# zhaotudou/HeteroFusionRCNN

Hardware: AMD Instinct MI355X
Metric: KITTI frames/sec RPN train step (higher is better)
Workload: dtype f32

## Files before the change

heterofusionrcnn_amd/csrc/xconv_common.h:

```cpp
#pragma once
#include "hf_common.h"

#include <initializer_list>

namespace hf {

template <int M>
__device__ __forceinline__ void store_m(float *base, size_t elem, const float (&v)[M])
{
    float *p = base + elem;
    if constexpr (M == 4 || M == 8) {
        if ((reinterpret_cast<uintptr_t>(base) & 15) == 0) {
#pragma unroll
            for (int q = 0; q < M / 4; ++q) reinterpret_cast<float4 *>(p)[q] = make_float4(v[4 * q], v[4 * q + 1], v[4 * q + 2], v[4 * q + 3]);
            return;
        }
    } else if constexpr (M == 2) {
        if ((reinterpret_cast<uintptr_t>(base) & 7) == 0) { *reinterpret_cast<float2 *>(p) = make_float2(v[0], v[1]); return; }
    }
#pragma unroll
    for (int m = 0; m < M; ++m) p[m] = v[m];
}
template <int M>
__device__ __forceinline__ void load_m(const float *base, size_t elem, float (&v)[M])
{
    const float *p = base + elem;
    if constexpr (M == 4 || M == 8) {
        if ((reinterpret_cast<uintptr_t>(base) & 15) == 0) {
#pragma unroll
            for (int q = 0; q < M / 4; ++q) {
                const float4 t = reinterpret_cast<const float4 *>(p)[q];
                v[4 * q] = t.x; v[4 * q + 1] = t.y; v[4 * q + 2] = t.z; v[4 * q + 3] = t.w;
            }
            return;
        }
    } else if constexpr (M == 2) {
        if ((reinterpret_cast<uintptr_t>(base) & 7) == 0) { const float2 t = *reinterpret_cast<const float2 *>(p); v[0] = t.x; v[1] = t.y; return; }
    }
#pragma unroll
    for (int m = 0; m < M; ++m) v[m] = p[m];
}


constexpr int kXcThreads = 256;

typedef float f2 __attribute__((ext_vector_type(2)));

struct XcPair {
    const float *base;
    unsigned hi;
    bool gathered, live, hi_live;
};

__device__ __forceinline__ XcPair xc_pair(int ch, int c, int c0, const float *f, const float *fts, bool gather)
{
    XcPair s;
    s.live = ch < c;
    s.hi_live = ch + 1 < c;
    const int cc = s.live ? ch : (c - 1) & ~1;
    s.hi = s.hi_live ? 1u : 0u;
    s.gathered = gather && cc >= c0;
    s.base = s.gathered ? fts + (cc - c0) : f + cc;
    return s;
}

template <bool V2>
__device__ __forceinline__ f2 ld_pair(const float *p, unsigned hi)
{
    if constexpr (V2) return *reinterpret_cast<const f2 *>(p);
    else return f2{p[0], p[hi]};
}

template <int M, bool V2>
__device__ __forceinline__ void st_pair_m(float *p, bool hi_live, const f2 (&v)[M])
{
    if constexpr (V2) {
#pragma unroll
        for (int q = 0; q < M; ++q) {
            const int e0 = 2 * q, e1 = 2 * q + 1;
            reinterpret_cast<f2 *>(p)[q] = f2{e0 < M ? v[e0].x : v[e0 - M].y, e1 < M ? v[e1].x : v[e1 - M].y};
        }
    } else {
#pragma unroll
        for (int m = 0; m < M; ++m) p[m] = v[m].x;
        if (hi_live) {
#pragma unroll
            for (int m = 0; m < M; ++m) p[M + m] = v[m].y;
        }
    }
}

constexpr int kXcRows = 2;

struct XcCloud {
    long long next;
    unsigned tbase;
};

__device__ __forceinline__ unsigned xc_tbase(XcCloud &cl, long long r, int rows_per_cloud, int n_src)
{
    while (r >= cl.next) { cl.next += rows_per_cloud; cl.tbase += static_cast<unsigned>(n_src); }
    return cl.tbase;
}

__device__ __forceinline__ XcCloud xc_cloud(long long r, int rows_per_cloud, int n_src)
{
    const long long b = r / rows_per_cloud;
    return XcCloud{(b + 1) * rows_per_cloud, static_cast<unsigned>(b * n_src)};
}

template <int K, bool GATHER, bool V2>
__device__ __forceinline__ void xc_gather_row(const XcPair &s, long long r, unsigned tbase, const int *__restrict__ idx,
                                              unsigned lstride, unsigned c1, f2 (&fv)[K])
{
    const unsigned rk = static_cast<unsigned>(r) * K;
#pragma unroll
    for (int j = 0; j < K; ++j) {
        const unsigned lo = (rk + j) * lstride;
        unsigned off = lo;
        if constexpr (GATHER) {
            const unsigned go = (tbase + static_cast<unsigned>(idx[rk + j])) * c1;
            off = s.gathered ? go : lo;
        }
        fv[j] = ld_pair<V2>(s.base + off, s.hi);
    }
}

template <int K>
struct XcXRows {
    static constexpr int KK = K * K, Q = (KK + 63) / 64;
    float v[kXcRows][Q];
    __device__ __forceinline__ void load(const float *__restrict__ x, const long long (&rr)[kXcRows], int lane)
    {
#pragma unroll
        for (int i = 0; i < kXcRows; ++i)
#pragma unroll
            for (int q = 0; q < Q; ++q) {
                const int p = lane + 64 * q;
                v[i][q] = x[rr[i] * KK + (p < KK ? p : KK - 1)];
            }
    }
    __device__ __forceinline__ void stage(float (*xs)[KK], int lane) const
    {
        __builtin_amdgcn_fence(__ATOMIC_SEQ_CST, "wavefront");
        __builtin_amdgcn_wave_barrier();
#pragma unroll
        for (int i = 0; i < kXcRows; ++i)
#pragma unroll
            for (int q = 0; q < Q; ++q)
                if (lane + 64 * q < KK) xs[i][lane + 64 * q] = v[i][q];
        __builtin_amdgcn_fence(__ATOMIC_SEQ_CST, "wavefront");
        __builtin_amdgcn_wave_barrier();
    }
};

struct XcSource {
    const float *base;
    long long stride;
    bool gathered;
};

__device__ __forceinline__ XcSource xc_source(int ch, int c, int c0, const float *f, const float *fts, const int *idx)
{
    XcSource s;
    if (idx == nullptr) { s.base = f + ch; s.stride = c; s.gathered = false; }
    else if (ch - (ch & 63) < c0) { s.base = f + ch; s.stride = c0; s.gathered = false; }
    else { s.base = fts + (ch - c0); s.stride = c - c0; s.gathered = true; }
    return s;
}


template <int K, int M, bool GATHER, bool V2, bool BN>
__global__ __launch_bounds__(kXcThreads) void xconv_dw_fwd_kernel(long long rows, int c, int c0, int rows_per_block,
                                                                 const float *__restrict__ x, const float *__restrict__ f,
                                                                 const float *__restrict__ gamma, const float *__restrict__ beta,
                                                                 const float *__restrict__ mean, const float *__restrict__ invstd,
                                                                 const float *__restrict__ fts, const int *__restrict__ idx, int n_src,
                                                                 int rows_per_cloud, const float *__restrict__ wd, float *__restrict__ out)
{
    static_assert(GATHER || !BN, "the BatchNorm fold exists on the gather route only");
    const int lane = threadIdx.x & 63, wave = __builtin_amdgcn_readfirstlane(static_cast<int>(threadIdx.x >> 6));
    const int ch = blockIdx.y * 128 + 2 * lane;
    const XcPair src = xc_pair(ch, c, c0, f, fts, GATHER);
    const int cw = src.live ? ch : (c - 1) & ~1;
    f2 w[K][M];
#pragma unroll
    for (int k = 0; k < K; ++k)
#pragma unroll
        for (int m = 0; m < M; ++m) w[k][m] = f2{wd[(static_cast<size_t>(k) * c + cw) * M + m], wd[(static_cast<size_t>(k) * c + cw + src.hi) * M + m]};
    bool some_lifted = false;
    f2 ba, bmu, bb;
    if constexpr (BN) {
        const int cb = src.gathered ? 0 : cw;
        some_lifted = static_cast<int>(blockIdx.y) * 128 < c0;
        ba = f2{gamma[cb] * invstd[cb], gamma[cb + 1] * invstd[cb + 1]};
        bmu = f2{mean[cb], mean[cb + 1]};
        bb = f2{beta[cb], beta[cb + 1]};
    }
    const unsigned lstride = GATHER ? c0 : c, c1 = c - c0;
    const long long r0 = static_cast<long long>(blockIdx.x) * rows_per_block;
    const long long r1 = r0 + rows_per_block < rows ? r0 + rows_per_block : rows;
    __shared__ float xs[kXcThreads / 64][kXcRows][K * K];
    XcCloud cl = xc_cloud(r0, rows_per_cloud, n_src);
    for (long long rb = r0 + wave; rb < r1; rb += 4 * kXcRows) {
        f2 fv[kXcRows][K];
        long long rr[kXcRows];
#pragma unroll
        for (int i = 0; i < kXcRows; ++i) rr[i] = rb + 4 * i < r1 ? rb + 4 * i : r1 - 1;
        XcXRows<K> xrow;
        xrow.load(x, rr, lane);
#pragma unroll
        for (int i = 0; i < kXcRows; ++i) {
            const unsigned tb = GATHER ? xc_tbase(cl, rr[i], rows_per_cloud, n_src) : 0u;
            xc_gather_row<K, GATHER, V2>(src, rr[i], tb, idx, lstride, c1, fv[i]);
        }
        xrow.stage(xs[wave], lane);
#pragma unroll
        for (int i = 0; i < kXcRows; ++i) {
            if (rb + 4 * i >= r1) break;
            if constexpr (BN) {
                if (some_lifted) {
#pragma unroll
                    for (int j = 0; j < K; ++j) {
                        const f2 z = fv[i][j];
                        const f2 h = ba * (f2{elu_stream(z.x), elu_stream(z.y)} - bmu) + bb;
                        fv[i][j] = src.gathered ? z : h;
                    }
                }
            }
            const float *xr = xs[wave][i];
            f2 o[M];
#pragma unroll
            for (int m = 0; m < M; ++m) o[m] = f2{0.f, 0.f};
#pragma unroll
            for (int k = 0; k < K; ++k) {
                f2 t = xr[k * K] * fv[i][0];
#pragma unroll
                for (int j = 1; j < K; ++j) t = t + xr[k * K + j] * fv[i][j];
#pragma unroll
                for (int m = 0; m < M; ++m) o[m] = o[m] + t * w[k][m];
            }
            if (src.live) st_pair_m<M, V2>(out + static_cast<size_t>(rr[i] * c + ch) * M, src.hi_live, o);
        }
    }
}

template <int K, int M, bool GATHER, bool BN>
__global__ __launch_bounds__(kXcThreads) __attribute__((amdgpu_waves_per_eu(BN ? 4 : 1))) void xconv_dw_bwd_fw_kernel(
    long long rows, int c, int c0, int rows_per_block, const float *__restrict__ x, const float *__restrict__ f,
    const float *__restrict__ gamma, const float *__restrict__ beta, const float *__restrict__ mean, const float *__restrict__ invstd,
    const float *__restrict__ fts, const int *__restrict__ idx, int n_src, int rows_per_cloud, const float *__restrict__ wd,
    const float *__restrict__ grad_out, float *__restrict__ grad_f, float *__restrict__ grad_gathered, float *__restrict__ grad_wd,
    float *__restrict__ wd_partial, float *__restrict__ bn_partial)
{
    static_assert(GATHER || !BN, "the BatchNorm fold exists on the gather route only");
    const int lane = threadIdx.x & 63, wave = __builtin_amdgcn_readfirstlane(static_cast<int>(threadIdx.x >> 6));
    const int ch = blockIdx.y * 64 + lane;
    const bool live = ch < c;
    const XcSource src = xc_source(live ? ch : blockIdx.y * 64, c, c0, f, fts, GATHER ? idx : nullptr);
    if (GATHER && src.gathered && !grad_wd && !grad_gathered) return;
    bool lifted = false;
    float bis, ba, bmu, bb, s1 = 0.f, s2 = 0.f;
    if constexpr (BN) {
        lifted = static_cast<int>(blockIdx.y) * 64 < c0;
        const int cb = lifted ? ch : 0;
        bis = invstd[cb]; ba = gamma[cb] * bis; bmu = mean[cb]; bb = beta[cb];
    }
    float w[K][M], gw[K][M];
#pragma unroll
    for (int k = 0; k < K; ++k)
#pragma unroll
        for (int m = 0; m < M; ++m) { w[k][m] = live ? wd[(static_cast<size_t>(k) * c + ch) * M + m] : 0.f; gw[k][m] = 0.f; }
    const long long r0 = static_cast<long long>(blockIdx.x) * rows_per_block;
    const long long r1 = r0 + rows_per_block < rows ? r0 + rows_per_block : rows;
    for (long long r = r0 + wave; r < r1; r += kXcThreads / 64) {
        const float *xr = x + r * (K * K);
        float fv[K], xv[K], g[M], gfx[K];
        const long long tbase = (GATHER && src.gathered) ? static_cast<long long>(static_cast<unsigned>(r) / static_cast<unsigned>(rows_per_cloud)) * n_src : 0;
#pragma unroll
        for (int j = 0; j < K; ++j) {
            const long long srow = (GATHER && src.gathered) ? tbase + idx[r * K + j] : r * K + j;
            fv[j] = live ? src.base[srow * src.stride] : 0.f;
            if constexpr (BN) xv[j] = 0.f;
        }
        if constexpr (BN) {
            if (lifted) {
#pragma unroll
                for (int j = 0; j < K; ++j) {
                    xv[j] = elu_stream(fv[j]);
                    fv[j] = ba * (xv[j] - bmu) + bb;
                }
            }
        }
        load_m<M>(grad_out, static_cast<size_t>(r * c + (live ? ch : 0)) * M, g);
        if (!live) {
#pragma unroll
            for (int m = 0; m < M; ++m) g[m] = 0.f;
        }
#pragma unroll
        for (int k = 0; k < K; ++k) {
            float a = 0.f;
#pragma unroll
            for (int m = 0; m < M; ++m) a = a + g[m] * w[k][m];
            gfx[k] = a;
            float t = xr[k * K] * fv[0];
#pragma unroll
            for (int j = 1; j < K; ++j) t = t + xr[k * K + j] * fv[j];
#pragma unroll
            for (int m = 0; m < M; ++m) gw[k][m] = gw[k][m] + t * g[m];
        }
        float *gdst = (GATHER && src.gathered) ? (grad_gathered ? grad_gathered + (ch - c0) : nullptr) : (grad_f ? grad_f + ch : nullptr);
        if (live && gdst) {
            float ga[K];
#pragma unroll
            for (int j = 0; j < K; ++j) {
                float a = xr[j] * gfx[0];
#pragma unroll
                for (int k = 1; k < K; ++k) a = a + xr[k * K + j] * gfx[k];
                gdst[(r * K + j) * src.stride] = a;
                ga[j] = a;
            }
            if constexpr (BN) {
                if (lifted) {
#pragma unroll
                    for (int j = 0; j < K; ++j) { s1 += ga[j]; s2 += ga[j] * ((xv[j] - bmu) * bis); }
                }
            }
        }
    }
    __shared__ float red[K * M][64];
    if constexpr (BN) {
        if (lifted && grad_f) {
            for (int wv = 0; wv < kXcThreads / 64; ++wv) {
                if (wave == wv) {
                    red[0][lane] = wv == 0 ? s1 : red[0][lane] + s1;
                    red[1][lane] = wv == 0 ? s2 : red[1][lane] + s2;
                }
                __syncthreads();
            }
            if (wave == 0) {
                float *mine = bn_partial + static_cast<size_t>(blockIdx.x) * 2 * c0;
                mine[ch] = red[0][lane];
                mine[c0 + ch] = red[1][lane];
            }
        }
    }
    if (grad_wd) {
        for (int wv = 0; wv < kXcThreads / 64; ++wv) {
            if (wave == wv && live) {
#pragma unroll
                for (int k = 0; k < K; ++k)
#pragma unroll
                    for (int m = 0; m < M; ++m) red[k * M + m][lane] = wv == 0 ? gw[k][m] : red[k * M + m][lane] + gw[k][m];
            }
            __syncthreads();
        }
        float *mine = (BN || wd_partial) ? wd_partial + static_cast<size_t>(blockIdx.x) * K * c * M : nullptr;
        for (int i = threadIdx.x; i < K * M * 64; i += kXcThreads) {
            const int km = i >> 6, c2 = blockIdx.y * 64 + (i & 63);
            if (c2 < c) {
                const size_t e = (static_cast<size_t>(km / M) * c + c2) * M + km % M;
                if (BN || mine) mine[e] = red[km][i & 63];
                else atomicAdd(&grad_wd[e], red[km][i & 63]);
            }
        }
    }
}


template <int M>
__device__ __forceinline__ void xc_load_m(const float *arg, const float *p, float (&v)[M])
{
    if constexpr (M == 4) {
        if ((reinterpret_cast<uintptr_t>(arg) & 15) == 0) {
            const float4 t = *reinterpret_cast<const float4 *>(p);
            v[0] = t.x; v[1] = t.y; v[2] = t.z; v[3] = t.w;
            return;
        }
    } else if constexpr (M == 2) {
        if ((reinterpret_cast<uintptr_t>(arg) & 7) == 0) { const float2 t = *reinterpret_cast<const float2 *>(p); v[0] = t.x; v[1] = t.y; return; }
    }
#pragma unroll
    for (int m = 0; m < M; ++m) v[m] = p[m];
}

struct XcCloudDiv {
    long long first, next;
    long long tbase;
};

__device__ __forceinline__ long long xc_tbase_div(XcCloudDiv &cl, long long r, int rows_per_cloud, int n_src)
{
    if (r >= cl.next || r < cl.first) {
        const long long b = static_cast<long long>(static_cast<unsigned>(r) / static_cast<unsigned>(rows_per_cloud));
        cl.first = b * rows_per_cloud;
        cl.next = cl.first + rows_per_cloud;
        cl.tbase = b * n_src;
    }
    return cl.tbase;
}

template <int CTRL>
__device__ __forceinline__ float xc_dpp(float v)
{
    return __int_as_float(__builtin_amdgcn_update_dpp(0, __float_as_int(v), CTRL, 0xf, 0xf, true));
}

template <int KK, int OFF, int N>
__device__ __forceinline__ void xc_lane_fold(float (&v)[KK], int lane)
{
    static_assert(N == 64 || N == 16, "chunks of 64 or 16 entries");
    typedef unsigned u2 __attribute__((ext_vector_type(2)));
#pragma unroll
    for (int i = 0; i < N / 2; ++i) {
        const u2 s = __builtin_amdgcn_permlane32_swap(__float_as_uint(v[OFF + i]), __float_as_uint(v[OFF + i + N / 2]), false, false);
        v[OFF + i] = __uint_as_float(s.x) + __uint_as_float(s.y);
    }
#pragma unroll
    for (int i = 0; i < N / 4; ++i) {
        const u2 s = __builtin_amdgcn_permlane16_swap(__float_as_uint(v[OFF + i]), __float_as_uint(v[OFF + i + N / 4]), false, false);
        v[OFF + i] = __uint_as_float(s.x) + __uint_as_float(s.y);
    }
    const bool b3 = (lane & 8) != 0, b2 = (lane & 4) != 0;
#pragma unroll
    for (int i = 0; i < N / 8; ++i) {
        const float lo = v[OFF + i], hi = v[OFF + i + N / 8];
        v[OFF + i] = (b3 ? hi : lo) + xc_dpp<0x128>(b3 ? lo : hi);
    }
#pragma unroll
    for (int i = 0; i < N / 16; ++i) {
        const float lo = v[OFF + i], hi = v[OFF + i + N / 16];
        v[OFF + i] = (b2 ? hi : lo) + xc_dpp<0x141>(b2 ? lo : hi);
    }
    if constexpr (N == 64) {
        const bool b1 = (lane & 2) != 0, b0 = (lane & 1) != 0;
#pragma unroll
        for (int i = 0; i < 2; ++i) {
            const float lo = v[OFF + i], hi = v[OFF + i + 2];
            v[OFF + i] = (b1 ? hi : lo) + xc_dpp<0x4e>(b1 ? lo : hi);
        }
        const float lo = v[OFF], hi = v[OFF + 1];
        v[OFF] = (b0 ? hi : lo) + xc_dpp<0xb1>(b0 ? lo : hi);
    } else {
        v[OFF] = v[OFF] + xc_dpp<0x4e>(v[OFF]);
        v[OFF] = v[OFF] + xc_dpp<0xb1>(v[OFF]);
    }
}

template <int KK, int OFF = 0>
__device__ __forceinline__ void xc_store_dx(float (&acc)[KK], int lane, float *__restrict__ dst)
{
    static_assert((KK - OFF) % 64 == 0 || (KK - OFF) % 64 == 16, "K * K is a multiple of 64, or 16 more");
    if constexpr (KK - OFF >= 64) {
        xc_lane_fold<KK, OFF, 64>(acc, lane);
        dst[OFF + lane] = acc[OFF];
        xc_store_dx<KK, OFF + 64>(acc, lane, dst);
    } else if constexpr (KK - OFF == 16) {
        xc_lane_fold<KK, OFF, 16>(acc, lane);
        if ((lane & 3) == 0) dst[OFF + (lane >> 2)] = acc[OFF];
    }
}

__device__ __forceinline__ const float *xc_at(const float *base, unsigned byte_off)
{
    return reinterpret_cast<const float *>(reinterpret_cast<const char *>(base) + byte_off);
}

constexpr int kXcWdSlots = 64;
inline __host__ __device__ bool xc_bwd_x_fast(int c, int km) { return ((c + 63) >> 6) * km <= kXcWdSlots; }
inline size_t xc_bwd_x_lds_bytes(int c, int c0_bn, int km)
{
    return xc_bwd_x_fast(c, km) ? sizeof(float) * (64 * static_cast<size_t>((c + 63) >> 6) * km + 3 * static_cast<size_t>(c0_bn)) : 0;
}

template <int K, int M>
struct XcTrip {
    float fv[K], g[M];
};

template <int K, int M, bool GATHER, bool BN, bool FAST>
__device__ __forceinline__ void xc_bwd_x_rows(long long rows, int c, int c0, const float *__restrict__ f,
                                              const float *__restrict__ gamma, const float *__restrict__ beta,
                                              const float *__restrict__ mean, const float *__restrict__ invstd,
                                              const float *__restrict__ fts, const int *__restrict__ idx, int n_src, int rows_per_cloud,
                                              const float *__restrict__ wd, const float *__restrict__ grad_out,
                                              float *__restrict__ grad_x, float *lds)
{
    constexpr int KK = K * K, KM = K * M;
    const int lane = threadIdx.x & 63, w = __builtin_amdgcn_readfirstlane(static_cast<int>(threadIdx.x >> 6));
    const long long wave = w + static_cast<long long>(blockIdx.x) * (kXcThreads / 64);
    const long long nwaves = static_cast<long long>(gridDim.x) * (kXcThreads / 64);
    const int trips = (c + 63) >> 6, c1 = c - c0;
    const unsigned lstride = GATHER ? c0 : c;
    float *bnl = lds + trips * KM * 64;
    if constexpr (FAST) {
        for (int i = threadIdx.x; i < trips * KM * 64; i += kXcThreads) {
            const int l = i & 63, s = i >> 6, t = s / KM, km = s - t * KM, ch = 64 * t + l;
            lds[i] = ch < c ? wd[(static_cast<size_t>(km / M) * c + ch) * M + km % M] : 0.f;
        }
        if constexpr (BN) {
            for (int i = threadIdx.x; i < c0; i += kXcThreads) {
                bnl[i] = gamma[i] * invstd[i];
                bnl[c0 + i] = mean[i];
                bnl[2 * c0 + i] = beta[i];
            }
        }
        __syncthreads();
    }
    if (wave >= rows) return;

    int nidx[K];
    auto load_idx = [&](long long r) {
        if constexpr (GATHER) {
            const long long rc = r < rows ? r : rows - 1;
#pragma unroll
            for (int j = 0; j < K; ++j) nidx[j] = idx[rc * K + j];
        }
    };
    XcCloudDiv cl{0, 0, 0};
    const float *fl = f, *go = grad_out, *tj[K];
    auto set_row = [&](long long r) {
        fl = f + r * K * static_cast<long long>(lstride);
        go = grad_out + r * c * static_cast<long long>(M);
        if constexpr (GATHER) {
            const long long tb = xc_tbase_div(cl, r, rows_per_cloud, n_src);
#pragma unroll
            for (int j = 0; j < K; ++j) tj[j] = fts + static_cast<unsigned long long>(tb + nidx[j]) * static_cast<unsigned>(c1);
        }
    };
    auto load_trip = [&](int t, XcTrip<K, M> &o) {
        const int ch = 64 * t + lane;
        const unsigned cc = ch < c ? ch : c - 1;
        const float *bj[K];
        unsigned sub = 0;
        if (GATHER && 64 * t >= c0) {
            sub = c0;
#pragma unroll
            for (int j = 0; j < K; ++j) bj[j] = tj[j];
        } else {
#pragma unroll
            for (int j = 0; j < K; ++j) bj[j] = fl + j * static_cast<size_t>(lstride);
        }
        const unsigned off = (cc - sub) * 4u;
#pragma unroll
        for (int j = 0; j < K; ++j) o.fv[j] = *xc_at(bj[j], off);
        xc_load_m<M>(grad_out, xc_at(go, cc * (4u * M)), o.g);
    };

    long long r = wave;
    int t = 0;
    load_idx(r);
    set_row(r);
    XcTrip<K, M> cur, nxt;
    load_trip(0, cur);
    static_assert(K % 2 == 0, "pairs of j");
    f2 acc[K][K / 2];
    for (;;) {
        const bool last = t + 1 == trips;
        const long long rn = last ? r + nwaves : r;
        const int tn = last ? 0 : t + 1;
        const bool more = rn < rows;
        if (t == 0) load_idx(r + nwaves);
        if (last) set_row(more ? rn : r);
        load_trip(tn, nxt);
        const int ch = 64 * t + lane;
        const bool live = ch < c;
        const unsigned cc = live ? ch : c - 1;
        if (BN && 64 * t < c0) {
            float ba, bmu, bb;
            if constexpr (FAST) { ba = bnl[cc]; bmu = bnl[c0 + cc]; bb = bnl[2 * c0 + cc]; }
            else { ba = gamma[cc] * invstd[cc]; bmu = mean[cc]; bb = beta[cc]; }
#pragma unroll
            for (int j = 0; j < K; ++j) cur.fv[j] = ba * (elu_stream(cur.fv[j]) - bmu) + bb;
        }
        f2 ap[K / 2];
        {
            const float *wt = lds + (t * KM * 64 + lane);
            auto wv = [&](int k, int m) { return FAST ? wt[(k * M + m) * 64] : wd[(static_cast<size_t>(k) * c + cc) * M + m]; };
#pragma unroll
            for (int i = 0; i < K / 2; ++i) {
                ap[i] = cur.g[0] * f2{wv(2 * i, 0), wv(2 * i + 1, 0)};
#pragma unroll
                for (int m = 1; m < M; ++m) ap[i] = ap[i] + cur.g[m] * f2{wv(2 * i, m), wv(2 * i + 1, m)};
            }
        }
        f2 fp[K / 2];
#pragma unroll
        for (int i = 0; i < K / 2; ++i) fp[i] = f2{cur.fv[2 * i], cur.fv[2 * i + 1]};
        if (t == 0) {
            if (live) {
#pragma unroll
                for (int k = 0; k < K; ++k)
#pragma unroll
                    for (int i = 0; i < K / 2; ++i) acc[k][i] = ap[k / 2][k % 2] * fp[i];
            } else {
#pragma unroll
                for (int k = 0; k < K; ++k)
#pragma unroll
                    for (int i = 0; i < K / 2; ++i) acc[k][i] = f2{0.f, 0.f};
            }
        } else if (live) {
#pragma unroll
            for (int k = 0; k < K; ++k) {
                f2 p[K / 2];
#pragma unroll
                for (int i = 0; i < K / 2; ++i) p[i] = ap[k / 2][k % 2] * fp[i];
                __builtin_amdgcn_sched_barrier(0);
#pragma unroll
                for (int i = 0; i < K / 2; ++i) acc[k][i] = acc[k][i] + p[i];
                __builtin_amdgcn_sched_barrier(0);
            }
        }
        if (last) {
            float flat[KK];
#pragma unroll
            for (int k = 0; k < K; ++k)
#pragma unroll
                for (int i = 0; i < K / 2; ++i) { flat[k * K + 2 * i] = acc[k][i].x; flat[k * K + 2 * i + 1] = acc[k][i].y; }
            xc_store_dx<KK>(flat, lane, grad_x + r * KK);
        }
        if (!more) break;
        cur = nxt;
        r = rn;
        t = tn;
    }
}

template <int K, int M, bool GATHER, bool BN>
__device__ __forceinline__ void xc_bwd_x_body(long long rows, int c, int c0, const float *__restrict__ f,
                                              const float *__restrict__ gamma, const float *__restrict__ beta,
                                              const float *__restrict__ mean, const float *__restrict__ invstd,
                                              const float *__restrict__ fts, const int *__restrict__ idx, int n_src, int rows_per_cloud,
                                              const float *__restrict__ wd, const float *__restrict__ grad_out,
                                              float *__restrict__ grad_x, float *lds)
{
    if (xc_bwd_x_fast(c, K * M))
        xc_bwd_x_rows<K, M, GATHER, BN, true>(rows, c, c0, f, gamma, beta, mean, invstd, fts, idx, n_src, rows_per_cloud, wd, grad_out, grad_x, lds);
    else
        xc_bwd_x_rows<K, M, GATHER, BN, false>(rows, c, c0, f, gamma, beta, mean, invstd, fts, idx, n_src, rows_per_cloud, wd, grad_out, grad_x, lds);
}

void xdw_pair_grid(long long rows, int c, dim3 &grid, int &rpb, int blocks_per_cu);
void xdw_bwd_grid(long long rows, int c, dim3 &grid, int &rpb);
bool xdw_offsets_fit(long long rows, int k, int c, long long src_rows);
bool xdw_v2(int c, std::initializer_list<const void *> ptrs);
bool xdw_fts_direct(long long rows, int n_src, int rows_per_cloud, int k, int c1, int m);
size_t xdw_gathered_bytes(int b, int rows_per_cloud, int k, int c1);
int xdw_table_grad(long long src_rows, int n_src, int rows_per_cloud, int k, int c, int c0, int m, const float *x, const float *wd,
                   const float *grad_out, const int *offsets, const int *entries, float *grad_fts, hipStream_t st);

struct XdwGradPlan {
    bool direct;
    float *gathered;
    float *wd_partial;
};
XdwGradPlan xdw_grad_plan(int b, int n_src, int rows_per_cloud, int k, int c1, int m, const float *grad_fts, void *workspace);
int xdw_grad_table(const XdwGradPlan &plan, int b, int n_src, int rows_per_cloud, int k, int c0, int c1, int m, const float *x,
                   const float *wd, const float *grad_out, const int *offsets, const int *entries, float *grad_fts, hf_stream_t stream);
int xdw_grad_empty(int b, int n_src, int k, int c0, int c1, int m, float *grad_fts, float *grad_wd, hipStream_t st);

}
```

Baseline: 332.3.

## Restructure depthwise weight-grad backward kernel with LDS-staged X and prefetched row batches

Rewrites the xconv depthwise backward (weight/feature grad) kernel so each wave stages its X matrices into LDS in paired layout. It processes k in pairs with packed f2 math, software-pipelines the gathered feature, index and grad_out loads one batch ahead, and uses scalar base pointers with unsigned lane offsets. Large K*M configurations keep weights in LDS, and the occupancy hint is raised to 4 waves/EU for all variants. The aim is to hide gather latency and cut address arithmetic and VGPR pressure, at the cost of extra LDS traffic, more complex code and possible register spills.

```diff
diff --git a/heterofusionrcnn_amd/csrc/xconv_common.h b/heterofusionrcnn_amd/csrc/xconv_common.h
--- a/heterofusionrcnn_amd/csrc/xconv_common.h
+++ b/heterofusionrcnn_amd/csrc/xconv_common.h
@@ -2,6 +2,7 @@
 #include "hf_common.h"
 
 #include <initializer_list>
+#include <type_traits>
 
 namespace hf {
 
@@ -103,6 +104,16 @@
     return cl.tbase;
 }
 
+__device__ __forceinline__ unsigned xc_tbase_step(XcCloud &cl, long long r, int rows_per_cloud, int n_src)
+{
+    while (r >= cl.next) {
+        cl.next += rows_per_cloud;
+        cl.tbase += static_cast<unsigned>(n_src);
+        asm volatile("" : "+s"(cl.tbase));
+    }
+    return cl.tbase;
+}
+
 __device__ __forceinline__ XcCloud xc_cloud(long long r, int rows_per_cloud, int n_src)
 {
     const long long b = r / rows_per_cloud;
@@ -168,6 +179,73 @@
     else { s.base = fts + (ch - c0); s.stride = c - c0; s.gathered = true; }
     return s;
 }
+
+__device__ __forceinline__ const float *xc_at(const float *base, unsigned byte_off)
+{
+    return reinterpret_cast<const float *>(reinterpret_cast<const char *>(base) + byte_off);
+}
+
+typedef __attribute__((address_space(1))) float xc_gfloat;
+__device__ __forceinline__ xc_gfloat *xc_sbase(const float *p)
+{
+    const unsigned long long b = reinterpret_cast<unsigned long long>(p);
+    unsigned lo = __builtin_amdgcn_readfirstlane(static_cast<unsigned>(b)), hi = __builtin_amdgcn_readfirstlane(static_cast<unsigned>(b >> 32));
+    asm("" : "+s"(lo), "+s"(hi));
+    return (xc_gfloat *)((static_cast<unsigned long long>(hi) << 32) | lo);
+}
+__device__ __forceinline__ unsigned xc_lane_off(unsigned off)
+{
+    asm volatile("" : "+v"(off));
+    return off;
+}
+__device__ __forceinline__ xc_gfloat *xc_gat(xc_gfloat *base, unsigned byte_off)
+{
+    return (xc_gfloat *)((__attribute__((address_space(1))) char *)base + byte_off);
+}
+
+template <int M>
+__device__ __forceinline__ void xc_load_m(const float *arg, const float *p, float (&v)[M])
+{
+    if constexpr (M == 4) {
+        if ((reinterpret_cast<uintptr_t>(arg) & 15) == 0) {
+            const float4 t = *reinterpret_cast<const float4 *>(p);
+            v[0] = t.x; v[1] = t.y; v[2] = t.z; v[3] = t.w;
+            return;
+        }
+    } else if constexpr (M == 2) {
+        if ((reinterpret_cast<uintptr_t>(arg) & 7) == 0) { const float2 t = *reinterpret_cast<const float2 *>(p); v[0] = t.x; v[1] = t.y; return; }
+    }
+#pragma unroll
+    for (int m = 0; m < M; ++m) v[m] = p[m];
+}
+
+template <int M>
+__device__ __forceinline__ void xc_gload_m(const float *arg, xc_gfloat *p, float (&v)[M])
+{
+    typedef float v4 __attribute__((ext_vector_type(4)));
+    if constexpr (M == 4) {
+        if ((reinterpret_cast<uintptr_t>(arg) & 15) == 0) {
+            const v4 t = *(__attribute__((address_space(1))) v4 *)p;
+            v[0] = t.x; v[1] = t.y; v[2] = t.z; v[3] = t.w;
+            return;
+        }
+    } else if constexpr (M == 2) {
+        if ((reinterpret_cast<uintptr_t>(arg) & 7) == 0) { const f2 t = *(__attribute__((address_space(1))) f2 *)p; v[0] = t.x; v[1] = t.y; return; }
+    }
+#pragma unroll
+    for (int m = 0; m < M; ++m) v[m] = p[m];
+}
+
+template <int K, int M, int R>
+struct XcFwBatch {
+    static constexpr int Q = (K * K + 63) / 64;
+    float x[R][Q];
+    f2 fv[R][K / 2];
+    float g[R][M];
+};
+constexpr int xc_fw_rows(int k, int m, bool bn) { return k * m >= 24 ? 1 : kXcRows; }
+constexpr bool xc_fw_wd_lds(int k, int m) { return k * m >= 32; }
+constexpr bool xc_fw_pipe(int k, int m, bool bn) { return k == 4 || k * m <= 8; }
 
 
 template <int K, int M, bool GATHER, bool V2, bool BN>
@@ -246,7 +324,7 @@
 }
 
 template <int K, int M, bool GATHER, bool BN>
-__global__ __launch_bounds__(kXcThreads) __attribute__((amdgpu_waves_per_eu(BN ? 4 : 1))) void xconv_dw_bwd_fw_kernel(
+__global__ __launch_bounds__(kXcThreads) __attribute__((amdgpu_waves_per_eu(4))) void xconv_dw_bwd_fw_kernel(
     long long rows, int c, int c0, int rows_per_block, const float *__restrict__ x, const float *__restrict__ f,
     const float *__restrict__ gamma, const float *__restrict__ beta, const float *__restrict__ mean, const float *__restrict__ invstd,
     const float *__restrict__ fts, const int *__restrict__ idx, int n_src, int rows_per_cloud, const float *__restrict__ wd,
@@ -254,6 +332,7 @@
     float *__restrict__ wd_partial, float *__restrict__ bn_partial)
 {
     static_assert(GATHER || !BN, "the BatchNorm fold exists on the gather route only");
+    constexpr int R = xc_fw_rows(K, M, BN), Q = XcFwBatch<K, M, R>::Q;
     const int lane = threadIdx.x & 63, wave = __builtin_amdgcn_readfirstlane(static_cast<int>(threadIdx.x >> 6));
     const int ch = blockIdx.y * 64 + lane;
     const bool live = ch < c;
@@ -266,69 +345,178 @@
         const int cb = lifted ? ch : 0;
         bis = invstd[cb]; ba = gamma[cb] * bis; bmu = mean[cb]; bb = beta[cb];
     }
-    float w[K][M], gw[K][M];
-#pragma unroll
-    for (int k = 0; k < K; ++k)
-#pragma unroll
-        for (int m = 0; m < M; ++m) { w[k][m] = live ? wd[(static_cast<size_t>(k) * c + ch) * M + m] : 0.f; gw[k][m] = 0.f; }
+    static_assert(K % 2 == 0, "pairs of k");
+    constexpr bool WL = xc_fw_wd_lds(K, M);
+    __shared__ float red[K * M][64];
+    f2 *const wl = reinterpret_cast<f2 *>(&red[0][0]) + lane * M;
+    f2 w[WL ? 1 : K / 2][M], gw[K / 2][M];
+#pragma unroll
+    for (int kp = 0; kp < K / 2; ++kp)
+#pragma unroll
+        for (int m = 0; m < M; ++m) {
+            const f2 wk = live ? f2{wd[(static_cast<size_t>(2 * kp) * c + ch) * M + m], wd[(static_cast<size_t>(2 * kp + 1) * c + ch) * M + m]} : f2{0.f, 0.f};
+            if constexpr (WL) { if (wave == 0) wl[kp * 64 * M + m] = wk; }
+            else w[kp][m] = wk;
+            gw[kp][m] = f2{0.f, 0.f};
+        }
+    if constexpr (WL) __syncthreads();
     const long long r0 = static_cast<long long>(blockIdx.x) * rows_per_block;
     const long long r1 = r0 + rows_per_block < rows ? r0 + rows_per_block : rows;
-    for (long long r = r0 + wave; r < r1; r += kXcThreads / 64) {
-        const float *xr = x + r * (K * K);
-        float fv[K], xv[K], g[M], gfx[K];
-        const long long tbase = (GATHER && src.gathered) ? static_cast<long long>(static_cast<unsigned>(r) / static_cast<unsigned>(rows_per_cloud)) * n_src : 0;
-#pragma unroll
-        for (int j = 0; j < K; ++j) {
-            const long long srow = (GATHER && src.gathered) ? tbase + idx[r * K + j] : r * K + j;
-            fv[j] = live ? src.base[srow * src.stride] : 0.f;
-            if constexpr (BN) xv[j] = 0.f;
-        }
+    const bool gathered = GATHER && static_cast<int>(blockIdx.y) * 64 >= c0;
+    const int cc = live ? ch : c - 1;
+    const unsigned stride = static_cast<unsigned>(GATHER ? (gathered ? c - c0 : c0) : c);
+    const unsigned foff = static_cast<unsigned>(gathered ? cc - c0 : cc) * 4u, goff = static_cast<unsigned>(cc) * (4u * M);
+    unsigned xoff[Q];
+#pragma unroll
+    for (int q = 0; q < Q; ++q) xoff[q] = static_cast<unsigned>(lane + 64 * q < K * K ? lane + 64 * q : K * K - 1) * 4u;
+    float *const gdst = gathered ? grad_gathered : grad_f;
+    __shared__ float xs[kXcThreads / 64][R][2][K * K];
+    unsigned xpos[Q];
+#pragma unroll
+    for (int q = 0; q < Q; ++q) {
+        const int e = lane + 64 * q < K * K ? lane + 64 * q : K * K - 1, k = e / K, j = e - k * K;
+        xpos[q] = ((k >> 1) * K + j) * 2 + (k & 1);
+    }
+    auto stage = [&](const float (&xr)[R][Q]) {
+        __builtin_amdgcn_fence(__ATOMIC_SEQ_CST, "wavefront");
+        __builtin_amdgcn_wave_barrier();
+#pragma unroll
+        for (int i = 0; i < R; ++i)
+#pragma unroll
+            for (int q = 0; q < Q; ++q)
+                if (lane + 64 * q < K * K) { xs[wave][i][0][xpos[q]] = xr[i][q]; xs[wave][i][1][lane + 64 * q] = xr[i][q]; }
+        __builtin_amdgcn_fence(__ATOMIC_SEQ_CST, "wavefront");
+        __builtin_amdgcn_wave_barrier();
+    };
+    XcCloud cl = xc_cloud(r0, rows_per_cloud, n_src);
+    constexpr bool PIPE = xc_fw_pipe(K, M, BN);
+    XcFwBatch<K, M, R> cur, nxt;
+    int nidx[R][K];
+    auto clamp_rows = [&](long long rb, long long (&rr)[R]) {
+#pragma unroll
+        for (int i = 0; i < R; ++i) rr[i] = rb + 4 * i < r1 ? rb + 4 * i : r1 - 1;
+    };
+    auto load_idx = [&](long long rb) __attribute__((always_inline)) {
+        if (gathered) {
+            long long rr[R];
+            clamp_rows(rb, rr);
+#pragma unroll
+            for (int i = 0; i < R; ++i)
+#pragma unroll
+                for (int j = 0; j < K; ++j) nidx[i][j] = idx[rr[i] * K + j];
+        }
+    };
+    auto issue = [&](long long rb, XcFwBatch<K, M, R> &o) __attribute__((always_inline)) {
+        long long rr[R];
+        clamp_rows(rb, rr);
+#pragma unroll
+        for (int i = 0; i < R; ++i) {
+            xc_gfloat *xb = xc_sbase(x + rr[i] * (K * K));
+#pragma unroll
+            for (int q = 0; q < Q; ++q) o.x[i][q] = *xc_gat(xb, xc_lane_off(xoff[q]));
+        }
+#pragma unroll
+        for (int i = 0; i < R; ++i) {
+            const unsigned fo = xc_lane_off(foff);
+            if (gathered) {
+                const unsigned tb = xc_tbase_step(cl, rr[i], rows_per_cloud, n_src);
+#pragma unroll
+                for (int j = 0; j < K; ++j)
+                    o.fv[i][j / 2][j % 2] = *xc_gat(xc_sbase(fts + static_cast<unsigned long long>(tb + static_cast<unsigned>(nidx[i][j])) * stride), fo);
+            } else {
+                const float *fl = f + rr[i] * K * static_cast<long long>(stride);
+#pragma unroll
+                for (int j = 0; j < K; ++j) o.fv[i][j / 2][j % 2] = *xc_gat(xc_sbase(fl + j * static_cast<size_t>(stride)), fo);
+            }
+            xc_gload_m<M>(grad_out, xc_gat(xc_sbase(grad_out + rr[i] * c * static_cast<long long>(M)), xc_lane_off(goff)), o.g[i]);
+        }
+    };
+    auto row = [&](auto ga_tag, const float *xr, long long r, const f2 (&fin)[K / 2], const float (&g)[M]) {
+        constexpr bool GA = decltype(ga_tag)::value;
+        f2 fv[K / 2], xv[K / 2];
+        float ga[K];
+#pragma unroll
+        for (int j = 0; j < K / 2; ++j) fv[j] = fin[j];
         if constexpr (BN) {
             if (lifted) {
 #pragma unroll
-                for (int j = 0; j < K; ++j) {
-                    xv[j] = elu_stream(fv[j]);
+                for (int j = 0; j < K / 2; ++j) {
+                    xv[j] = f2{elu_stream(fv[j].x), elu_stream(fv[j].y)};
                     fv[j] = ba * (xv[j] - bmu) + bb;
                 }
             }
         }
-        load_m<M>(grad_out, static_cast<size_t>(r * c + (live ? ch : 0)) * M, g);
-        if (!live) {
-#pragma unroll
-            for (int m = 0; m < M; ++m) g[m] = 0.f;
-        }
-#pragma unroll
-        for (int k = 0; k < K; ++k) {
-            float a = 0.f;
-#pragma unroll
-            for (int m = 0; m < M; ++m) a = a + g[m] * w[k][m];
-            gfx[k] = a;
-            float t = xr[k * K] * fv[0];
-#pragma unroll
-            for (int j = 1; j < K; ++j) t = t + xr[k * K + j] * fv[j];
-#pragma unroll
-            for (int m = 0; m < M; ++m) gw[k][m] = gw[k][m] + t * g[m];
-        }
-        float *gdst = (GATHER && src.gathered) ? (grad_gathered ? grad_gathered + (ch - c0) : nullptr) : (grad_f ? grad_f + ch : nullptr);
-        if (live && gdst) {
-            float ga[K];
-#pragma unroll
-            for (int j = 0; j < K; ++j) {
-                float a = xr[j] * gfx[0];
-#pragma unroll
-                for (int k = 1; k < K; ++k) a = a + xr[k * K + j] * gfx[k];
-                gdst[(r * K + j) * src.stride] = a;
-                ga[j] = a;
+        const f2 *xp = reinterpret_cast<const f2 *>(xr), *xn = reinterpret_cast<const f2 *>(xr + K * K);
+        f2 gap[K / 2];
+#pragma unroll
+        for (int kp = 0; kp < K / 2; ++kp) {
+            f2 a = f2{0.f, 0.f};
+#pragma unroll
+            for (int m = 0; m < M; ++m) a = a + g[m] * (WL ? wl[kp * 64 * M + m] : w[WL ? 0 : kp][m]);
+            f2 t = xp[kp * K] * fv[0].x;
+#pragma unroll
+            for (int j = 1; j < K; ++j) t = t + xp[kp * K + j] * fv[j / 2][j % 2];
+#pragma unroll
+            for (int m = 0; m < M; ++m) {
+                gw[kp][m] = gw[kp][m] + t * g[m];
+                asm volatile("" : "+v"(gw[kp][m]));
+            }
+            if constexpr (GA) {
+#pragma unroll
+                for (int jp = 0; jp < K / 2; ++jp) gap[jp] = kp == 0 ? xn[jp] * a.x : gap[jp] + xn[2 * kp * (K / 2) + jp] * a.x;
+#pragma unroll
+                for (int jp = 0; jp < K / 2; ++jp) gap[jp] = gap[jp] + xn[(2 * kp + 1) * (K / 2) + jp] * a.y;
+            }
+            __builtin_amdgcn_sched_barrier(0);
+        }
+        if constexpr (GA) {
+#pragma unroll
+            for (int jp = 0; jp < K / 2; ++jp) { ga[2 * jp] = gap[jp].x; ga[2 * jp + 1] = gap[jp].y; }
+            float *gd = gdst + r * K * static_cast<long long>(stride);
+#pragma unroll
+            for (int j = 0; j < K; ++j) asm volatile("" : "+v"(ga[j]));
+            const unsigned fo = xc_lane_off(foff);
+            if (live) {
+#pragma unroll
+                for (int j = 0; j < K; ++j) *xc_gat(xc_sbase(gd + j * static_cast<size_t>(stride)), fo) = ga[j];
             }
             if constexpr (BN) {
                 if (lifted) {
 #pragma unroll
-                    for (int j = 0; j < K; ++j) { s1 += ga[j]; s2 += ga[j] * ((xv[j] - bmu) * bis); }
+                    for (int j = 0; j < K; ++j) { s1 += ga[j]; s2 += ga[j] * ((xv[j / 2][j % 2] - bmu) * bis); }
                 }
             }
         }
-    }
-    __shared__ float red[K * M][64];
+    };
+    auto run = [&](auto ga_tag) __attribute__((always_inline)) {
+        const long long rb0 = r0 + wave;
+        if (rb0 < r1) {
+            load_idx(rb0);
+            if constexpr (PIPE) {
+                issue(rb0, cur);
+                load_idx(rb0 + 4 * R);
+            }
+        }
+        for (long long rb = rb0; rb < r1; rb += 4 * R) {
+            if constexpr (PIPE) {
+                issue(rb + 4 * R, nxt);
+                load_idx(rb + 8 * R);
+            } else {
+                issue(rb, cur);
+                load_idx(rb + 4 * R);
+            }
+            stage(cur.x);
+#pragma unroll
+            for (int i = 0; i < R; ++i) {
+                if (rb + 4 * i >= r1) break;
+                row(ga_tag, xs[wave][i][0], rb + 4 * i, cur.fv[i], cur.g[i]);
+            }
+            if constexpr (PIPE) cur = nxt;
+        }
+    };
+    if (gdst) run(std::true_type{});
+    else run(std::false_type{});
+    if constexpr (WL) __syncthreads();
     if constexpr (BN) {
         if (lifted && grad_f) {
             for (int wv = 0; wv < kXcThreads / 64; ++wv) {
@@ -351,7 +539,7 @@
 #pragma unroll
                 for (int k = 0; k < K; ++k)
 #pragma unroll
-                    for (int m = 0; m < M; ++m) red[k * M + m][lane] = wv == 0 ? gw[k][m] : red[k * M + m][lane] + gw[k][m];
+                    for (int m = 0; m < M; ++m) red[k * M + m][lane] = wv == 0 ? gw[k / 2][m][k % 2] : red[k * M + m][lane] + gw[k / 2][m][k % 2];
             }
             __syncthreads();
         }
@@ -367,22 +555,6 @@
     }
 }
 
-
-template <int M>
-__device__ __forceinline__ void xc_load_m(const float *arg, const float *p, float (&v)[M])
-{
-    if constexpr (M == 4) {
-        if ((reinterpret_cast<uintptr_t>(arg) & 15) == 0) {
-            const float4 t = *reinterpret_cast<const float4 *>(p);
-            v[0] = t.x; v[1] = t.y; v[2] = t.z; v[3] = t.w;
-            return;
-        }
-    } else if constexpr (M == 2) {
-        if ((reinterpret_cast<uintptr_t>(arg) & 7) == 0) { const float2 t = *reinterpret_cast<const float2 *>(p); v[0] = t.x; v[1] = t.y; return; }
-    }
-#pragma unroll
-    for (int m = 0; m < M; ++m) v[m] = p[m];
-}
 
 struct XcCloudDiv {
     long long first, next;
@@ -459,11 +631,6 @@
         xc_lane_fold<KK, OFF, 16>(acc, lane);
         if ((lane & 3) == 0) dst[OFF + (lane >> 2)] = acc[OFF];
     }
-}
-
-__device__ __forceinline__ const float *xc_at(const float *base, unsigned byte_off)
-{
-    return reinterpret_cast<const float *>(reinterpret_cast<const char *>(base) + byte_off);
 }
 
 constexpr int kXcWdSlots = 64;
```

New measurement: 336.9 (median of 6 runs). 1.01x the previous value.
